# aleCombi/Hedgehog.jl

Hardware: AMD Instinct MI355X
Metric: MC path-steps/sec (Heston Euler-Maruyama, 1e6 paths x 252 steps per GPU) (higher is better)
Workload: dtype f64

## Files before the change

### hedgehog.jl_amd/csrc/hh_api.hip

```cpp
#include <cmath>
#include <cstdarg>
#include <cstdio>
#include <cstring>
#include <mutex>
#include <vector>

#include "hh_kernels.h"

#include "hh_ctx.h"

namespace {

const char* const kNoCtx = "hedgehog_mc: no context";

int ncomp_of(int dynamics) { return dynamics == HH_HESTON ? 2 : 1; }

constexpr uint64_t kMaxPaths = (1ull << 32) - 256;
constexpr uint32_t kMaxEulerSteps = 4u * 65535u;
constexpr uint32_t kMaxGridSteps = 65534u;

static bool bk_law_ok(const hh_model* m, double dt) {
  const double s2 = m->sigma * m->sigma;
  const double d = 4.0 * m->kappa * m->theta / s2;
  if (!(d >= 1e-8 && d <= 1e6)) return false;
  const double em1 = -std::expm1(-m->kappa * dt);
  const double lam_per_v = 4.0 * m->kappa * std::exp(-m->kappa * dt) / (s2 * em1);
  const double cscale = s2 * em1 / (4.0 * m->kappa);
  const double nuk = 4.0 * m->kappa * std::exp(-0.5 * m->kappa * dt) / s2 / em1;
  return std::isfinite(lam_per_v) && lam_per_v >= 0.0 && std::isfinite(cscale) && cscale > 0.0 &&
         std::isfinite(nuk) && nuk > 0.0 && std::isfinite(m->kappa * (1.0 + std::exp(-m->kappa * dt)) / em1);
}

int validate(hh_ctx* ctx, const hh_model* m, const hh_config* c) {
  if (!m || !c) return fail(ctx, HH_ERR_INVALID, "model/config is NULL");
  if (c->n_paths == 0) return fail(ctx, HH_ERR_INVALID, "n_paths must be >= 1");
  if (c->n_paths > kMaxPaths)
    return fail(ctx, HH_ERR_INVALID, "n_paths too large (max 2^32 - 256 per call; shard the ensemble)");
  if (c->strategy == HH_EULER_MARUYAMA && c->n_steps > kMaxEulerSteps)
    return fail(ctx, HH_ERR_INVALID, "n_steps too large (max %u)", kMaxEulerSteps);
  if (c->n_partials > HH_MAX_PARTIALS)
    return fail(ctx, HH_ERR_INVALID, "n_partials %u > HH_MAX_PARTIALS", c->n_partials);
  const bool logn = c->dynamics == HH_LOGNORMAL, hest = c->dynamics == HH_HESTON;
  if (!logn && !hest) return fail(ctx, HH_ERR_INVALID, "unknown dynamics %d", c->dynamics);
  const bool ok = (logn && (c->strategy == HH_EULER_MARUYAMA || c->strategy == HH_EXACT_LAW)) ||
                  (hest && (c->strategy == HH_EULER_MARUYAMA || c->strategy == HH_BROADIE_KAYA));
  if (!ok)
    return fail(ctx, HH_ERR_UNSUPPORTED, "no simulation method for dynamics %d with strategy %d",
                c->dynamics, c->strategy);
  if (!(m->S0 > 0.0) || !std::isfinite(m->S0)) return fail(ctx, HH_ERR_INVALID, "S0 must be > 0");
  if (!(m->T > 0.0) || !std::isfinite(m->T)) return fail(ctx, HH_ERR_INVALID, "T must be > 0");
  if (m->cp != 1.0 && m->cp != -1.0) return fail(ctx, HH_ERR_INVALID, "cp must be +1 or -1");
  if (hest && !(std::fabs(m->rho) <= 1.0)) return fail(ctx, HH_ERR_INVALID, "|rho| must be <= 1");
  if (!std::isfinite(m->sigma) || !std::isfinite(m->r_drift) || !std::isfinite(m->discount) ||
      !std::isfinite(m->strike) ||
      (hest && (!std::isfinite(m->V0) || !std::isfinite(m->kappa) || !std::isfinite(m->theta))))
    return fail(ctx, HH_ERR_INVALID, "model scalars must be finite");
  if (c->strategy == HH_EULER_MARUYAMA && c->n_steps == 0)
    return fail(ctx, HH_ERR_INVALID, "n_steps must be >= 1 for EulerMaruyama");
  if (c->strategy == HH_BROADIE_KAYA) {
    if (c->antithetic)
      return fail(ctx, HH_ERR_UNSUPPORTED, "HestonBroadieKaya has no antithetic form");
    if (c->n_partials)
      return fail(ctx, HH_ERR_UNSUPPORTED, "HestonBroadieKaya does not carry dual partials");
    if (m->sigma == 0.0 || m->kappa == 0.0 || !(m->V0 > 0.0))
      return fail(ctx, HH_ERR_INVALID, "HestonBroadieKaya needs sigma != 0, kappa != 0, V0 > 0");
    if ((c->bk_root_form != HH_BK_ROOT_SECANT && c->bk_root_form != HH_BK_ROOT_ORDER2) ||
        (c->bk_bracket_form != HH_BK_BRACKET_MIDPOINT && c->bk_bracket_form != HH_BK_BRACKET_ROOTS) ||
        (c->bk_caps != HH_BK_CAPS_AS_WRITTEN && c->bk_caps != HH_BK_CAPS_ROOTS_DEFAULT))
      return fail(ctx, HH_ERR_INVALID, "bk_root_form, bk_bracket_form, bk_caps: 0 or 1 each (hedgehog_mc.h)");
    if (!bk_law_ok(m, m->T))
      return fail(ctx, HH_ERR_INVALID, "HestonBroadieKaya needs 1e-8 <= d = 4 kappa theta / sigma^2 <= 1e6 "
                                       "(Bessel order d/2 - 1 strictly above -1, tables up to order 5e5) and "
                                       "finite transition constants (|kappa T| < 700)");
  }
  const bool euler = c->strategy == HH_EULER_MARUYAMA;
  if (c->noise_mode == HH_NOISE_REPLAY) {
    if (!c->replay) return fail(ctx, HH_ERR_INVALID, "REPLAY needs a replay buffer");
    if (((uintptr_t)c->replay & 15u) != 0)
      return fail(ctx, HH_ERR_INVALID, "replay buffer must be 16-byte aligned");
    if (c->replay_len) {
      uint64_t need = c->n_paths;
      if (c->strategy == HH_BROADIE_KAYA) need = 3 * c->n_paths;
// ... 320 lines not shown
    p.records = ctx->frecords;
    p.accum = accum_dev;
    fused_controls(ctx, p);
  }
  if (reduced) *reduced = fuse || bk;
  if (bk) {
    rc = ensure_bk_scratch(ctx, hh::bk_scratch_bytes(c->n_paths, ctx->bk_term_cache));
    if (rc) return rc;
    p.accum = accum_dev ? accum_dev : ctx->accum;
    p.bk_scratch = ctx->bk_scratch;
    p.bk_table_key = &ctx->bk_table_key;
    p.bk_term_cache = ctx->bk_term_cache;
    ctx->bk_last_n = c->n_paths;
    ctx->bk_last_cache = ctx->bk_term_cache;
  }

  if ((rc = stage_noise(ctx, c, p, false))) return rc;

  const size_t n_term = (size_t)c->n_paths * (c->antithetic ? 2 : 1);
  if (terminal && c->terminal_on_device) {
    p.terminal = terminal;
  } else if (terminal || need_terminal_dev) {
    rc = ensure(ctx, ctx->terminal, n_term);
    if (rc) return rc;
    p.terminal = ctx->terminal;
  }
  const int n_active = c->n_partials ? hh::count_active_partials(*m, *c) : 0;
  if (need_terminal_dev && n_active) {
    rc = ensure(ctx, ctx->terminal_d, n_term * (size_t)hh::pad_partials((uint32_t)n_active));
    if (rc) return rc;
    p.terminal_d = ctx->terminal_d;
  }
  if (terminal_dev_out) *terminal_dev_out = p.terminal;

  if (ctx->timing) HH_HIP(ctx, hipEventRecord(ctx->tev[ctx->t_count % hh_ctx::kTimingSlots][0], ctx->stream));
  if (c->strategy == HH_BROADIE_KAYA)
    HH_HIP(ctx, hh::launch_bk(*m, *c, p, ctx->stream));
  else
    HH_HIP(ctx, hh::launch_simulation(*m, *c, p, ctx->stream));
  return HH_OK;
}

static int end_timing(hh_ctx* ctx) {
  if (ctx->timing) {
    HH_HIP(ctx, hipEventRecord(ctx->tev[ctx->t_count % hh_ctx::kTimingSlots][1], ctx->stream));
    ++ctx->t_count;
  }
  return HH_OK;
}

static int copy_back_terminal(hh_ctx* ctx, const hh_config* c, double* terminal) {
  if (terminal && !c->terminal_on_device) {
    const size_t n_term = (size_t)c->n_paths * (c->antithetic ? 2 : 1);
    HH_HIP(ctx, hipMemcpyAsync(terminal, ctx->terminal, n_term * sizeof(double),
                               hipMemcpyDeviceToHost, ctx->stream));
    HH_HIP(ctx, hipStreamSynchronize(ctx->stream));
  }
  return HH_OK;
}

int hh_mc_accumulate(hh_ctx* ctx, const hh_model* m, const hh_config* c, double* accum_dev,
                     double* terminal) {
  if (!ctx) return HH_ERR_INVALID;
  std::lock_guard<std::recursive_mutex> lock__(ctx->mu);
  int rc = validate(ctx, m, c);
  if (rc) return rc;
  if (!accum_dev) return fail(ctx, HH_ERR_INVALID, "accum_dev is NULL");
  HH_HIP(ctx, hipSetDevice(ctx->device));
  bool reduced = false;
  rc = run_simulation(ctx, m, c, terminal, false, nullptr, accum_dev, &reduced);
  if (rc) return rc;
  if (!reduced)
    HH_HIP(ctx, hh::launch_reduce_records(ctx->records, hh::sim_records(*c), (double)c->n_paths, accum_dev, ctx->stream, 1, m, c));
  if ((rc = end_timing(ctx))) return rc;
  if ((rc = release_host_operands(ctx))) return rc;
  return copy_back_terminal(ctx, c, terminal);
}

static int next_pass(int remaining) {
  if (remaining <= hh::kMaxModelsPerPass) return remaining;
  return remaining == hh::kMaxModelsPerPass + 1 ? hh::kMaxModelsPerPass - 1 : hh::kMaxModelsPerPass;
}

int hh_mc_accumulate_multi(hh_ctx* ctx, const hh_model* models, uint32_t n_models, const hh_config* c,
                           double* accum_dev, double* const* terminals) {
  if (!ctx) return HH_ERR_INVALID;
  std::lock_guard<std::recursive_mutex> lock__(ctx->mu);
  if (!models || n_models == 0 || n_models > HH_MAX_MODELS)
    return fail(ctx, HH_ERR_INVALID, "hh_mc_accumulate_multi: 1 .. %d models", HH_MAX_MODELS);
  if (!accum_dev) return fail(ctx, HH_ERR_INVALID, "accum_dev is NULL");
  int rc;
  for (uint32_t k = 0; k < n_models; ++k)
    if ((rc = validate(ctx, &models[k], c))) return rc;
  if (c->n_partials)
    return fail(ctx, HH_ERR_UNSUPPORTED, "several models in one pass carry no dual partials (n_partials must be 0)");
  if (n_models == 1) return hh_mc_accumulate(ctx, models, c, accum_dev, terminals ? terminals[0] : nullptr);
  HH_HIP(ctx, hipSetDevice(ctx->device));
  if (c->strategy == HH_BROADIE_KAYA) {
    const uint32_t count = hh::bk_record_count(c->n_paths);
    if ((rc = ensure(ctx, ctx->records, 2 * (size_t)count * hh::kRecStride))) return rc;
    std::vector<int> leader(n_models, -1);
    for (uint32_t k = 0; k < n_models; ++k)
      for (uint32_t j = 0; j < k; ++j)
        if (leader[j] < 0 && hh::bk_same_chain(models[j], models[k])) {
          leader[k] = (int)j;
          break;
        }
    for (uint32_t k = 0; k < n_models; ++k) {
      if (leader[k] >= 0) continue;
      if ((rc = hh_mc_accumulate(ctx, &models[k], c, accum_dev + (size_t)k * HH_ACC_LEN, terminals ? terminals[k] : nullptr)))
        return rc;
      for (uint32_t f = k + 1; f < n_models; ++f) {
        if (leader[f] != (int)k) continue;
        double* terminal = terminals ? terminals[f] : nullptr;
        hh::DevicePtrs p{};
        p.records = ctx->records + (size_t)count * hh::kRecStride;
        p.bk_scratch = ctx->bk_scratch;
        p.bk_term_cache = ctx->bk_term_cache;
        if (terminal && c->terminal_on_device) {
          p.terminal = terminal;
        } else if (terminal) {
          if ((rc = ensure(ctx, ctx->terminal, (size_t)c->n_paths))) return rc;
          p.terminal = ctx->terminal;
        }
        if (ctx->timing) HH_HIP(ctx, hipEventRecord(ctx->tev[ctx->t_count % hh_ctx::kTimingSlots][0], ctx->stream));
        HH_HIP(ctx, hh::launch_bk_refinish(models[f], *c, p, ctx->records, ctx->stream));
        HH_HIP(ctx, hh::launch_reduce_records(p.records, count, (double)c->n_paths, accum_dev + (size_t)f * HH_ACC_LEN,
                                              ctx->stream, 1, &models[f], c, false,
                                              hh::bk_live_records(ctx->bk_scratch, c->n_paths)));
        if ((rc = end_timing(ctx))) return rc;
        if ((rc = copy_back_terminal(ctx, c, terminal))) return rc;
      }
    }
    return HH_OK;
  }
  const uint32_t n_tiles = hh::tiles_for(c->n_paths);
  const size_t rec_elems = (size_t)n_tiles * hh::kRecStride;
  const bool fuse = fuse_for(ctx, c);
  if (fuse) rc = ensure_poisoned(ctx, (size_t)n_models * rec_elems);
  else rc = ensure(ctx, ctx->records, (size_t)n_models * rec_elems);
  if (rc) return rc;
  hh::DevicePtrs base{};
  if (fuse) fused_controls(ctx, base);
  if ((rc = stage_noise(ctx, c, base, true))) return rc;
  const size_t n_term = (size_t)c->n_paths * (c->antithetic ? 2 : 1);
  bool any_host_terminal = false;
  if (terminals && !c->terminal_on_device) {
    for (uint32_t k = 0; k < n_models; ++k) any_host_terminal = any_host_terminal || terminals[k] != nullptr;
    if (any_host_terminal && (rc = ensure(ctx, ctx->terminal, (size_t)n_models * n_term))) return rc;
  }
  std::vector<hh::DevicePtrs> p(n_models, base);
  for (uint32_t k = 0; k < n_models; ++k) {
    p[k].records = (fuse ? ctx->frecords : ctx->records) + (size_t)k * rec_elems;
    p[k].accum = fuse ? accum_dev + (size_t)k * HH_ACC_LEN : nullptr;
    double* t = terminals ? terminals[k] : nullptr;
    p[k].terminal = !t ? nullptr : c->terminal_on_device ? t : ctx->terminal + (size_t)k * n_term;
  }
  if (ctx->timing) HH_HIP(ctx, hipEventRecord(ctx->tev[ctx->t_count % hh_ctx::kTimingSlots][0], ctx->stream));
  for (uint32_t k0 = 0; k0 < n_models;) {
    const int take = next_pass((int)(n_models - k0));
    HH_HIP(ctx, hh::launch_simulation_multi(models + k0, take, *c, p.data() + k0, ctx->stream));
    if (!fuse)
      for (int k = 0; k < take; ++k)
        HH_HIP(ctx, hh::launch_reduce_records(p[k0 + k].records, hh::sim_records(*c), (double)c->n_paths,
                                              accum_dev + (size_t)(k0 + k) * HH_ACC_LEN, ctx->stream, 1, &models[k0 + k], c));
    k0 += (uint32_t)take;
  }
  if ((rc = end_timing(ctx))) return rc;
  if ((rc = release_host_operands(ctx))) return rc;
  if (any_host_terminal) {
    for (uint32_t k = 0; k < n_models; ++k)
      if (terminals[k])
        HH_HIP(ctx, hipMemcpyAsync(terminals[k], p[k].terminal, n_term * sizeof(double), hipMemcpyDeviceToHost, ctx->stream));
    HH_HIP(ctx, hipStreamSynchronize(ctx->stream));
  }
  return HH_OK;
}

int hh_mc_solve_multi(hh_ctx* ctx, const hh_model* models, uint32_t n_models, const hh_config* c, hh_result* out,
                      double* const* terminals) {
  if (!ctx) return HH_ERR_INVALID;
  std::lock_guard<std::recursive_mutex> lock__(ctx->mu);
  if (!out || !models || n_models == 0 || n_models > HH_MAX_MODELS)
    return fail(ctx, HH_ERR_INVALID, "hh_mc_solve_multi: 1 .. %d models and their results", HH_MAX_MODELS);
  const WallClock clock;
  HH_HIP(ctx, hipSetDevice(ctx->device));
  const size_t n_acc = (size_t)n_models * HH_ACC_LEN;
  int rc = ensure(ctx, ctx->basket_accum, n_acc);
  if (rc) return rc;
  HH_HIP(ctx, hipEventRecord(ctx->ev0, ctx->stream));
  if ((rc = hh_mc_accumulate_multi(ctx, models, n_models, c, ctx->basket_accum, terminals))) return rc;
  HH_HIP(ctx, hipEventRecord(ctx->ev1, ctx->stream));
  double host[HH_MAX_MODELS * HH_ACC_LEN];
  HH_HIP(ctx, hipMemcpyAsync(host, ctx->basket_accum, n_acc * sizeof(double), hipMemcpyDeviceToHost, ctx->stream));
  HH_HIP(ctx, hipStreamSynchronize(ctx->stream));
  double kernel_ms, total_ms;
  if ((rc = solve_times(ctx, clock, &kernel_ms, &total_ms))) return rc;
  rc = finalize_results(models, 1, c, host, n_models, kernel_ms, total_ms, out);
  return rc ? finalize_failed(ctx, rc) : HH_OK;
}

int hh_mc_accumulate_basket(hh_ctx* ctx, const hh_model* m, const hh_config* c,
                            const double* strikes, const double* cps, uint32_t n_payoffs,
                            double* accum_dev, double* terminal) {
  if (!ctx) return HH_ERR_INVALID;
  std::lock_guard<std::recursive_mutex> lock__(ctx->mu);
  int rc = validate(ctx, m, c);
  if (rc) return rc;
  if (!accum_dev || !strikes || !cps || n_payoffs == 0 || n_payoffs > 65535)
    return fail(ctx, HH_ERR_INVALID, "hh_mc_accumulate_basket: bad arguments");
  for (uint32_t k = 0; k < n_payoffs; ++k)
    if (cps[k] != 1.0 && cps[k] != -1.0) return fail(ctx, HH_ERR_INVALID, "cp must be +1 or -1");
  if (m->dstrike)
    return fail(ctx, HH_ERR_UNSUPPORTED, "strike partials are not carried through a basket");
  HH_HIP(ctx, hipSetDevice(ctx->device));
  double* term_dev = nullptr;
  rc = run_simulation(ctx, m, c, terminal, true, &term_dev);
  if (rc) return rc;

  hh::BasketArgs b{};
  b.n_paths = c->n_paths;
  b.n_chunks = hh::basket_chunks(c->n_paths);
  b.antithetic = c->antithetic;
  std::vector<double> payoffs(strikes, strikes + n_payoffs);
  payoffs.insert(payoffs.end(), cps, cps + n_payoffs);
  const double* payoffs_dev = nullptr;
  rc = stage_host(ctx, ctx->payoffs, payoffs.size(), payoffs.data(), payoffs.size(), &payoffs_dev);
  if (rc) return rc;
  rc = ensure(ctx, ctx->basket_records, (size_t)n_payoffs * b.n_chunks * hh::kRecStride);
  if (rc) return rc;
  b.terminal = term_dev;
  const int n_active = c->n_partials ? hh::count_active_partials(*m, *c) : 0;
  b.terminal_d = n_active ? ctx->terminal_d : nullptr;
  b.strikes = payoffs_dev;
  b.cps = payoffs_dev + n_payoffs;
  b.records = ctx->basket_records;
  HH_HIP(ctx, hh::launch_basket_payoffs(b, n_payoffs, (uint32_t)n_active, ctx->stream));
  HH_HIP(ctx, hh::launch_reduce_records(ctx->basket_records, b.n_chunks, (double)c->n_paths,
                                        accum_dev, ctx->stream, n_payoffs, m, c, true));
  if (c->strategy == HH_BROADIE_KAYA)
    HH_HIP(ctx, hh::launch_copy_bk_counters(ctx->accum, accum_dev, n_payoffs, ctx->stream));
  if ((rc = end_timing(ctx))) return rc;
  if ((rc = release_host_operands(ctx))) return rc;
  return copy_back_terminal(ctx, c, terminal);
}

int hh_mc_solve_basket(hh_ctx* ctx, const hh_model* m, const hh_config* c, const double* strikes,
                       const double* cps, uint32_t n_payoffs, hh_result* out, double* terminal) {
  if (!ctx) return HH_ERR_INVALID;
// ... 1033 lines not shown
```

### hedgehog.jl_amd/csrc/hh_kernels.h

```cpp
#pragma once
#include <hip/hip_runtime.h>
#include <stdint.h>

#include "../../include/hedgehog_mc.h"
#include "hh_layout.h"

namespace hh {

constexpr int kRecStride = HH_ACC_LEN;
constexpr unsigned long long kPoison = 0x7FF8C0DE7FF8C0DEull;
constexpr unsigned long long kFinishSpinTicksDefault = 500000000ull;
constexpr int kRecItmS = 11;

template <int P>
struct DualT {
  double v;
  double d[P > 0 ? P : 1];
};

constexpr int kMaxBasis = 4;
enum { kBasisV0 = 0, kBasisKappa = 1, kBasisTheta = 2, kBasisSigma = 3 };
struct PartialMap {
  int sim;
  int n;
// ... 5 lines not shown
};
template <int P>
struct SimArgs {
  DualT<P> x0;
  DualT<P> v0;
  DualT<P> kappa, theta, sigma;
  DualT<P> r;
  DualT<P> gdrift;
  DualT<P> strike;
  DualT<P> law_mu, law_sd;
  double dt, sqrt_dt, rho, rho_c, cp;
  uint64_t n_paths;
  uint64_t path_offset;
  uint32_t n_steps;
  uint32_t n_tiles;
  uint32_t tail_from;
  const uint64_t* seeds;
  const double* replay;
  double* terminal;
  double* terminal_d;
  double* records;
  double* accum;
  double acc_n_paths;
  unsigned int* finish_state;
  unsigned long long finish_spin_ticks;
  uint32_t reducer_tile;
  PartialMap map;
};

struct DevicePtrs {
  const uint64_t* seeds;
  const double* replay;
  double* terminal;
  double* terminal_d;
  double* records;
  double* accum;
  unsigned int* finish_state;
  long long finish_spin_ticks = -1;
  int finish_tile_first = 0;
  void* bk_scratch;
  struct BkTableKey* bk_table_key;
  int bk_term_cache;
  void* bk_sort;
  bool replay_path_major;
};
inline bool replay_direct_path_major(uint32_t n_steps, int ncomp) { return ((uint64_t)n_steps * ncomp) % 2 == 0; }
struct BkTableKey {
  const void* where;
  double nu;
  double kappa, sigma2, T;
};

constexpr int kBasketChunk = 4096;
struct BasketArgs {
  const double* terminal;
  const double* terminal_d;
  const double* strikes;
  const double* cps;
  uint64_t n_paths;
  uint32_t n_chunks;
  int antithetic;
  double* records;
};
inline uint32_t basket_chunks(uint64_t n_paths) {
  return (uint32_t)((n_paths + kBasketChunk - 1) / kBasketChunk);
}

constexpr int kExactPairs = 8, kExactPairsHuge = 64;
constexpr int kExactPairsSmall = 4;
int exact_pairs_per_lane(uint64_t n_paths);
inline uint32_t exact_records(uint64_t n_paths) {
  const uint64_t per = 512ull * (uint64_t)exact_pairs_per_lane(n_paths);
  return (uint32_t)((n_paths + per - 1) / per);
}
inline uint32_t sim_records(const hh_config& c) {
  return c.strategy == HH_EXACT_LAW ? exact_records(c.n_paths) : tiles_for(c.n_paths);
}
inline int pad_partials(uint32_t p) { return p <= 4 ? (int)p : 4; }

int launch_simulation(const hh_model& m, const hh_config& c, const DevicePtrs& p, hipStream_t s);
int launch_simulation_multi(const hh_model* models, int n_models, const hh_config& c, const DevicePtrs* p,
                            hipStream_t s);
constexpr int kMaxModelsPerPass = 4;
SimArgs<0> make_args0(const hh_model& m, const hh_config& c, const DevicePtrs& p);
struct BkTransition {
  const double* in_spot;
  const double* in_var;
  double* out_spot;
  double* out_var;
  uint32_t step;
};
bool bk_same_chain(const hh_model& a, const hh_model& b);
int launch_bk_refinish(const hh_model& m, const hh_config& c, const DevicePtrs& p, const double* rec0, hipStream_t s);
int launch_bk(const hh_model& m, const hh_config& c, const DevicePtrs& p, hipStream_t s,
              const BkTransition* tr = nullptr, bool upload_tables = true);
int launch_bk_grid(const hh_model& m, const hh_config& c, const DevicePtrs& p, hipStream_t s,
                   double* spot_rows, double* var_rows, uint32_t k0, uint32_t n_dates, bool upload_tables);
uint32_t bk_grid_dates_per_chain(uint64_t n_paths, uint32_t n_steps);
size_t bk_grid_sort_bytes(uint64_t n_chain);
size_t bk_scratch_bytes(uint64_t n_paths, int term_cache = 0);
void bk_diag_ptrs(const void* scratch, uint64_t n_paths, int term_cache, const uint32_t** decisions,
                  const uint32_t** series_len);
uint32_t bk_record_count(uint64_t n_paths);
const uint32_t* bk_live_records(const void* scratch, uint64_t n_paths);
int launch_copy_bk_counters(const double* src, double* accum, uint32_t n_groups, hipStream_t s);
int launch_fill_rows(double* spot0, double* var0, uint64_t n, double S0, double V0, hipStream_t s);
int launch_reduce_records(const double* records, uint32_t n_records, double n_paths, double* accum,
                          hipStream_t s, uint32_t n_groups = 1, const hh_model* m = nullptr,
                          const hh_config* c = nullptr, bool basket = false,
                          const uint32_t* n_records_dev = nullptr);
int count_active_partials(const hh_model& m, const hh_config& c);
int launch_basket_payoffs(const BasketArgs& b, uint32_t n_payoffs, uint32_t n_active_partials,
                          hipStream_t s);
constexpr uint32_t kCarrMadanMaxSubpanels = 1024;
uint32_t carr_madan_subpanels(double alpha, double bound);
int launch_carr_madan(const hh_model& m, int dynamics, int compat_sqrt_alpha, double alpha,
                      double bound, double* out_dev, hipStream_t s);
int launch_carr_madan_grad(const hh_model& m, int dynamics, int compat_sqrt_alpha, double alpha,
                           double bound, const double* per_payoff_dev, uint32_t n_payoffs,
                           double* out_dev, hipStream_t s);
int launch_carr_madan_basket(const hh_model& m, int dynamics, int compat_sqrt_alpha, double alpha,
                             double bound, const double* per_payoff_dev, uint32_t n_payoffs,
                             double* out_dev, hipStream_t s);
struct CrrTree {
  double F, K, cp, u, p, q, disc;
  int32_t style;
  uint32_t row;
};
int launch_crr(const CrrTree* trees_dev, const double* spot_factors_dev, int steps, uint32_t n_trees,
               double* out_dev, hipStream_t s);
struct FdOption {
  double S0, K, cp, r, T;
  double h, x0;
  double lo, di, up;
  int32_t style;
  int32_t pad_;
};
int launch_fd(const FdOption* opts_dev, int space_steps, int time_steps, int rannacher_steps, uint32_t n_options,
              double* out_dev, hipStream_t s);
uint32_t lsm_chunks(uint64_t ntot);
size_t lsm_scratch_doubles(uint64_t ntot, uint32_t n_steps, int degree);
enum { kLsmPhaseStats = 0, kLsmPhasePow = 1, kLsmPhaseInit = 2, kLsmPhaseStep = 3, kLsmPhaseFinal = 4 };
int launch_lsm_phase(int phase, uint32_t t, const double* grid, uint64_t ntot, uint32_t n_steps,
                     double strike, double cp, double step_discount, int degree, int32_t* tau,
                     double* val, double* scratch, double* records, const double* vec_in,
                     double* vec_out, hipStream_t s);
int launch_gbm_grid(const uint64_t* seeds_dev, uint64_t n_paths, uint32_t n_steps, double S0,
                    double r, double sigma, double T, int anti, double* grid, hipStream_t s);
int launch_euler_grid(const hh_model& m, const hh_config& c, const uint64_t* seeds_dev, bool log_state,
                      double* grid, double* var_grid, hipStream_t s);
int launch_path_stats(const hh_model& m, const hh_config& c, const uint64_t* seeds_dev, uint32_t monitor_every,
                      bool include_start, bool bridge, double* stats, hipStream_t s);
struct PathPayoffArgs {
  const double* stats;
  const hh_path_payoff* payoffs;
  double* values;
  double* records;
  double n_mon;
  uint64_t n_paths;
  uint32_t n_chunks;
  int antithetic;
  int extremes;
};
int launch_path_payoffs(const PathPayoffArgs& b, uint32_t n_payoffs, hipStream_t s);
double merton_compensator(const hh_jump& jump);
constexpr int kMertonPerLane = 8;
// ... 22 lines not shown
```

### hedgehog.jl_amd/csrc/hh_multi.hip

```cpp
#include <type_traits>

#include "hh_sim.h"

namespace hh {

template <int K>
struct MultiArgs {
  SimArgs<0> m[K];
};

constexpr int kMultiChunk = 4;
constexpr int kMultiMaxWaves = 3;

template <class M, bool REPLAY, bool ANTI, int K, bool SHARED>
__global__ __launch_bounds__(kTile)
__attribute__((amdgpu_waves_per_eu(1, REPLAY ? kMultiMaxWaves : 8))) void euler_multi_kernel(const MultiArgs<K> a) {
  constexpr int NC = M::NCOMP;
  using State = typename M::State;
  const SimArgs<0>& a0 = a.m[0];
  const uint32_t tile = blockIdx.x, tid = threadIdx.x;
  const uint64_t path = (uint64_t)tile * kTile + tid;
  const uint32_t n_steps = a0.n_steps;

  State st[K];
  State sa[ANTI ? K : 1];
#pragma unroll
  for (int k = 0; k < K; ++k) {
    M::init(st[k], a.m[k]);
    if constexpr (ANTI) M::init(sa[k], a.m[k]);
  }
  auto step_all = [&](double d1, double d2) {
#pragma unroll
    for (int k = 0; k < K; ++k) {
      M::step(st[k], a.m[k], d1, d2);
      if constexpr (ANTI) M::step(sa[k], a.m[k], -d1, -d2);
    }
  };

  if constexpr (REPLAY) {
    const double* __restrict__ base = a0.replay + (size_t)tile * n_steps * NC * kTile + tid;
    constexpr int CH = kMultiChunk;
    double X[CH][NC], Y[CH][NC];
    auto ld = [&](double(&buf)[CH][NC], uint32_t s0) {
#pragma unroll
      for (int u = 0; u < CH; ++u) {
        if (s0 + u < n_steps) {
#pragma unroll
          for (int c = 0; c < NC; ++c) buf[u][c] = stream_load(base + ((size_t)(s0 + u) * NC + c) * kTile);
        }
      }
    };
    auto go = [&](const double(&buf)[CH][NC], uint32_t s0) {
#pragma unroll
      for (int u = 0; u < CH; ++u)
        if (s0 + u < n_steps) step_all(buf[u][0], NC > 1 ? buf[u][NC - 1] : 0.0);
    };
    auto ldf = [&](double(&buf)[CH][NC], uint32_t s0) {
#pragma unroll
      for (int u = 0; u < CH; ++u)
#pragma unroll
        for (int c = 0; c < NC; ++c) buf[u][c] = stream_load(base + ((size_t)(s0 + u) * NC + c) * kTile);
    };
    auto gof = [&](const double(&buf)[CH][NC]) {
#pragma unroll
      for (int u = 0; u < CH; ++u) step_all(buf[u][0], NC > 1 ? buf[u][NC - 1] : 0.0);
    };
    uint32_t s = 0;
    if (n_steps >= 2u * CH) {
      ldf(X, 0);
      while (s + 3u * CH <= n_steps) {
        ldf(Y, s + CH);
        gof(X);
        ldf(X, s + 2u * CH);
        gof(Y);
        s += 2u * CH;
      }
      ld(Y, s + CH);
      gof(X);
      s += CH;
      ld(X, s + CH);
      go(Y, s);
      go(X, s + CH);
    } else {
      ld(X, 0);
      while (s < n_steps) {
        ld(Y, s + CH);
        go(X, s);
        s += CH;
        if (s >= n_steps) break;
        ld(X, s + CH);
        go(Y, s);
        s += CH;
      }
    }
  } else {
    const uint64_t key = path < a0.n_paths ? a0.seeds[path] : 0ull;
    if constexpr (NC == 2) {
      for (uint32_t s = 0; s < n_steps; ++s) {
        double z1, z2;
        normal_pair(key, s, 0u, 0u, kDomEuler, z1, z2);
        if constexpr (SHARED) {
          step_all(a0.sqrt_dt * z1, a0.sqrt_dt * fma(a0.rho, z1, a0.rho_c * z2));
        } else {
#pragma unroll
          for (int k = 0; k < K; ++k) {
            const double d1 = a.m[k].sqrt_dt * z1;
            const double d2 = a.m[k].sqrt_dt * fma(a.m[k].rho, z1, a.m[k].rho_c * z2);
            M::step(st[k], a.m[k], d1, d2);
            if constexpr (ANTI) M::step(sa[k], a.m[k], -d1, -d2);
          }
        }
      }
    } else {
      auto one = [&](double z) {
#pragma unroll
        for (int k = 0; k < K; ++k) {
          const double d = a.m[k].sqrt_dt * z;
          M::step(st[k], a.m[k], d, 0.0);
          if constexpr (ANTI) M::step(sa[k], a.m[k], -d, 0.0);
        }
      };
      for (uint32_t s = 0; s < n_steps; s += 2) {
        double z1, z2;
        normal_pair(key, s >> 1, 0u, 0u, kDomEuler, z1, z2);
        one(z1);
        if (s + 1 < n_steps) one(z2);
      }
    }
  }

#pragma unroll
  for (int k = 0; k < K; ++k) {
    double acc[4] = {0.0, 0.0, 0.0, 0.0};
    finish_path<0, ANTI>(st[k], sa[ANTI ? k : 0], a.m[k], path, acc);
    if (k) __syncthreads();
    block_reduce_publish<4, kTile / 64, 2>(acc, a.m[k].records + (size_t)tile * kRecStride, a.m[k].accum != nullptr, false);
  }
  if (a0.accum && reduces_records(tile, a0)) {
#pragma unroll
    for (int k = 0; k < K; ++k) {
      if (k) __syncthreads();
      finish_records<kTile, 0>(a.m[k]);
    }
  }
}

template <bool REPLAY, bool ANTI, int K, int PAIRS>
__global__ __launch_bounds__(kTile) void exact_multi_kernel(const MultiArgs<K> a) {
  const SimArgs<0>& a0 = a.m[0];
  const uint32_t chunk = blockIdx.x, tid = threadIdx.x;
  struct S {
    DualT<0> x;
  };
  double acc[K][4];
#pragma unroll
  for (int k = 0; k < K; ++k)
#pragma unroll
    for (int i = 0; i < 4; ++i) acc[k][i] = 0.0;
#pragma unroll 2
  for (int jp = 0; jp < PAIRS; ++jp) {
    const uint64_t path0 = ((uint64_t)chunk * PAIRS + jp) * (2 * kTile) + (uint64_t)tid * 2;
    double z[2];
    exact_pair_normals<REPLAY>(a0, path0, z);
#pragma unroll
    for (int k = 0; k < K; ++k) {
#pragma unroll
      for (int j = 0; j < 2; ++j) {
        S st, sa;
        st.x.v = fma(a.m[k].law_sd.v, z[j], a.m[k].law_mu.v);
        if constexpr (ANTI) sa.x.v = 2 * a.m[k].law_mu.v - st.x.v;
        finish_path<0, ANTI>(st, sa, a.m[k], path0 + j, acc[k]);
      }
    }
  }
#pragma unroll
  for (int k = 0; k < K; ++k) {
    if (k) __syncthreads();
    block_reduce_publish<4, kTile / 64, 2>(acc[k], a.m[k].records + (size_t)chunk * kRecStride, a.m[k].accum != nullptr, false);
  }
  if (a0.accum && reduces_records(chunk, a0)) {
#pragma unroll
    for (int k = 0; k < K; ++k) {
      if (k) __syncthreads();
      finish_records<kTile, 0>(a.m[k]);
    }
  }
}


template <class M, bool REPLAY, bool ANTI, int K>
static int launch_multi_k(const MultiArgs<K>& a, bool shared, hipStream_t s) {
  const dim3 g(a.m[0].n_tiles), b(kTile);
  if constexpr (!REPLAY && M::NCOMP == 2) {
    if (shared) {
      hipLaunchKernelGGL((euler_multi_kernel<M, REPLAY, ANTI, K, true>), g, b, 0, s, a);
      return (int)hipGetLastError();
    }
  }
  hipLaunchKernelGGL((euler_multi_kernel<M, REPLAY, ANTI, K, false>), g, b, 0, s, a);
  return (int)hipGetLastError();
}

template <class M, int K>
static int launch_multi_m(const MultiArgs<K>& a, bool replay, bool anti, bool shared, hipStream_t s) {
  if (replay) return anti ? launch_multi_k<M, true, true, K>(a, shared, s) : launch_multi_k<M, true, false, K>(a, shared, s);
  return anti ? launch_multi_k<M, false, true, K>(a, shared, s) : launch_multi_k<M, false, false, K>(a, shared, s);
}

template <int K>
static int launch_multi(const hh_model* models, const hh_config& c, const DevicePtrs* p, hipStream_t s) {
  MultiArgs<K> a;
  bool shared = true;
  for (int k = 0; k < K; ++k) {
    a.m[k] = make_args0(models[k], c, p[k]);
    shared = shared && a.m[k].rho == a.m[0].rho && a.m[k].dt == a.m[0].dt;
  }
  const bool anti = c.antithetic != 0, replay = c.noise_mode == HH_NOISE_REPLAY;
  if (c.strategy == HH_EXACT_LAW) {
    const dim3 g(a.m[0].n_tiles), b(kTile);
    auto pick = [&](auto replay_c, auto anti_c) {
      constexpr bool R = decltype(replay_c)::value, A = decltype(anti_c)::value;
      const int pairs = exact_pairs_per_lane(c.n_paths);
      return pairs == kExactPairsHuge ? exact_multi_kernel<R, A, K, kExactPairsHuge>
             : pairs == kExactPairs   ? exact_multi_kernel<R, A, K, kExactPairs>
                                      : exact_multi_kernel<R, A, K, kExactPairsSmall>;
    };
    using T = std::true_type;
    using F = std::false_type;
    auto kernel = replay ? (anti ? pick(T{}, T{}) : pick(T{}, F{})) : (anti ? pick(F{}, T{}) : pick(F{}, F{}));
    hipLaunchKernelGGL(kernel, g, b, 0, s, a);
    return (int)hipGetLastError();
  }
  if (c.dynamics == HH_LOGNORMAL) return launch_multi_m<GbmModel<0>, K>(a, replay, anti, shared, s);
  if (c.em_split) return launch_multi_m<HestonModel<0, true>, K>(a, replay, anti, shared, s);
  return launch_multi_m<HestonModel<0, false>, K>(a, replay, anti, shared, s);
}

int launch_simulation_multi(const hh_model* models, int n_models, const hh_config& c, const DevicePtrs* p,
                            hipStream_t s) {
  switch (n_models) {
    case 2: return launch_multi<2>(models, c, p, s);
    case 3: return launch_multi<3>(models, c, p, s);
    case 4: return launch_multi<4>(models, c, p, s);
    default: return (int)hipErrorInvalidValue;
  }
}

}
```

### hedgehog.jl_amd/csrc/hh_sim.h

```cpp
#pragma once
#include <type_traits>

#include "hh_kernels.h"
#include "hh_reduce.h"
#include "hh_rng.h"

namespace hh {


__device__ __forceinline__ double sqrt_clipped(double w) {
  const double y = __builtin_fmin(__builtin_amdgcn_rsq(w), 0x1p1000);
  double g = w * y, h = 0.5 * y;
  const double r = fma(-h, g, 0.5);
  g = fma(g, r, g);
  h = fma(h, r, h);
  g = fma(fma(-g, g, w), h, g);
  return fma(fma(-g, g, w), h, g);
}

template <int P, bool SPLIT>
struct HestonModel {
  static constexpr int NCOMP = 2;
  struct State {
    DualT<P> x, v;
  };
  __device__ static __forceinline__ void init(State& s, const SimArgs<P>& a) {
    s.x = a.x0;
    s.v = a.v0;
  }
  __device__ static __forceinline__ void step(State& s, const SimArgs<P>& a, double dW1,
                                              double dW2) {
    double g;
    step(s, a, dW1, dW2, g);
  }
  __device__ static __forceinline__ void step(State& s, const SimArgs<P>& a, double dW1, double dW2, double& g) {
    const bool pos = s.v.v > 0.0;
    double vp;
    asm("v_max_f64 %0, %1, 0" : "=v"(vp) : "v"(s.v.v));
    const double th_m_v = a.theta.v - vp;
    const double Kx = fma(a.dt, fma(-0.5, vp, a.r.v), s.x.v);
    const double Kv = fma(a.dt, a.kappa.v * th_m_v, s.v.v);
    const bool wpos = SPLIT ? (Kv > 0.0) : pos;
    const double w = SPLIT ? (wpos ? Kv : 0.0) : vp;
    const double sq = sqrt_clipped(w);
    if constexpr (P > 0) {
      double inv2s = 0.0;
      if (wpos) {
        const double r0 = __builtin_amdgcn_rcp(sq);
        inv2s = 0.5 * fma(r0, fma(-sq, r0, 1.0), r0);
      }
      const double A = a.dt * th_m_v, B = sq * dW2;
      const double m = pos ? 1.0 - a.dt * a.kappa.v : 1.0;
      const double h = pos ? 0.5 * a.dt : 0.0;
      const double e1 = inv2s * dW1;
      const double se2 = (a.sigma.v * inv2s) * dW2;
#pragma unroll
      for (int k = 0; k < P; ++k) {
        const double dv = s.v.d[k];
        const double f = fma(a.kappa.d[k], A, (a.dt * a.kappa.v) * a.theta.d[k]);
        const double Kvd = fma(m, dv, f);
        const double x0 = s.x.d[k] + a.dt * a.r.d[k];
        if constexpr (SPLIT) {
          s.x.d[k] = fma(e1, Kvd, fma(-h, dv, x0));
          s.v.d[k] = fma(se2, Kvd, fma(a.sigma.d[k], B, Kvd));
        } else {
          s.x.d[k] = fma(e1 - h, dv, x0);
          s.v.d[k] = fma(se2, dv, fma(a.sigma.d[k], B, Kvd));
        }
      }
    }
    s.x.v = fma(sq, dW1, Kx);
    s.v.v = fma(a.sigma.v * sq, dW2, Kv);
    g = sq;
  }
};

template <int P>
struct GbmModel {
  static constexpr int NCOMP = 1;
  struct State {
    DualT<P> x;
  };
  __device__ static __forceinline__ void init(State& s, const SimArgs<P>& a) { s.x = a.x0; }
  __device__ static __forceinline__ void step(State& s, const SimArgs<P>& a, double dW, double) {
    if constexpr (P > 0) {
#pragma unroll
      for (int k = 0; k < P; ++k)
        s.x.d[k] = fma(a.sigma.d[k], dW, fma(a.dt, a.gdrift.d[k], s.x.d[k]));
    }
    s.x.v = fma(a.sigma.v, dW, fma(a.dt, a.gdrift.v, s.x.v));
  }
  __device__ static __forceinline__ void step(State& s, const SimArgs<P>& a, double dW, double, double& g) {
    step(s, a, dW, 0.0);
    g = a.sigma.v;
  }
};


template <int P>
__device__ __forceinline__ void euler_pair_increments(uint64_t key, uint32_t s, const SimArgs<P>& a, double& d1,
                                                      double& d2) {
  double z1, z2;
  normal_pair(key, s, 0u, 0u, kDomEuler, z1, z2);
  d1 = a.sqrt_dt * z1;
  d2 = a.sqrt_dt * fma(a.rho, z1, a.rho_c * z2);
}
__device__ __forceinline__ void euler_scalar_normals(uint64_t key, uint32_t h, double& z1, double& z2) {
  normal_pair(key, h, 0u, 0u, kDomEuler, z1, z2);
}

__device__ __forceinline__ void euler_bridge_draws(uint64_t key, uint32_t k, double& L1, double& L2) {
  const Philox4 b = philox4x32_10(k, 0u, 0u, kDomBridge, (uint32_t)key, (uint32_t)(key >> 32));
  L1 = neg2_log_unit(u01_fast(b.c0, b.c1));
  L2 = neg2_log_unit(u01_fast(b.c2, b.c3));
}


template <int P>
__device__ __forceinline__ void payoff_of(const DualT<P>& x, const SimArgs<P>& a, double& S,
                                          double& p, double (&pd)[P > 0 ? P : 1], double& wS,
                                          double& wN) {
  S = exp(x.v);
  const double m = a.cp * (S - a.strike.v);
  const bool itm = m > 0.0;
  p = itm ? m : 0.0;
  wS = itm ? a.cp * S : 0.0;
  wN = itm ? a.cp : 0.0;
  if constexpr (P > 0) {
#pragma unroll
    for (int k = 0; k < P; ++k) pd[k] = wS * x.d[k];
  }
}

template <int N, int NWAVES, int TAIL = 0>
__device__ __forceinline__ void block_reduce_store(double (&acc)[N], double* __restrict__ rec) {
#pragma unroll
  for (int i = 0; i < N; ++i) {
#pragma unroll
    for (int off = 32; off > 0; off >>= 1) acc[i] += __shfl_down(acc[i], off, 64);
  }
  __shared__ double sm[NWAVES][N];
  const int lane = threadIdx.x & 63, wave = threadIdx.x >> 6;
  if (lane == 0) {
#pragma unroll
    for (int i = 0; i < N; ++i) sm[wave][i] = acc[i];
  }
  __syncthreads();
  if (threadIdx.x == 0) {
#pragma unroll
    for (int i = 0; i < kRecStride; ++i) rec[i] = 0.0;
#pragma unroll
    for (int i = 0; i < N; ++i) {
      double t = sm[0][i];
#pragma unroll
      for (int w = 1; w < NWAVES; ++w) t += sm[w][i];
      rec[i < N - TAIL ? i : kRecItmS + (i - (N - TAIL))] = t;
// ... 294 lines not shown
```

Before: 436.9 billion.

## Share one variance path across multi-model Heston passes with identical variance parameters

Adds a shared-variance kernel variant: when all models in a pass share v0, kappa, theta, sigma and dt (plus rho and noise when not replaying), the variance process is stepped once and only the log-spot update runs per model. Host-side pass planning groups models with identical variance processes into the same pass and sends single leftovers to the single-model kernel. This removes redundant sqrt and variance arithmetic per model per step, at the cost of more kernel instantiations, a tighter waves-per-EU bound for the replay variant, and a different pass partition.

```diff
diff --git a/hedgehog.jl_amd/csrc/hh_api.hip b/hedgehog.jl_amd/csrc/hh_api.hip
--- a/hedgehog.jl_amd/csrc/hh_api.hip
+++ b/hedgehog.jl_amd/csrc/hh_api.hip
@@ -1,3 +1,4 @@
+#include <algorithm>
 #include <cmath>
 #include <cstdarg>
 #include <cstdio>
@@ -484,6 +485,42 @@
   return remaining == hh::kMaxModelsPerPass + 1 ? hh::kMaxModelsPerPass - 1 : hh::kMaxModelsPerPass;
 }
 
+static std::vector<std::vector<uint32_t>> plan_passes(const hh_model* models, uint32_t n_models, const hh_config* c) {
+  using Pass = std::vector<uint32_t>;
+  auto cut = [](const Pass& of, std::vector<Pass>& into) {
+    for (size_t k0 = 0; k0 < of.size();) {
+      const size_t take = (size_t)next_pass((int)(of.size() - k0));
+      into.emplace_back(of.begin() + (long)k0, of.begin() + (long)(k0 + take));
+      k0 += take;
+    }
+  };
+  std::vector<Pass> groups;
+  for (uint32_t k = 0; k < n_models; ++k) {
+    size_t g = 0;
+    while (g < groups.size() && !hh::euler_same_variance(models[groups[g][0]], models[k], *c)) ++g;
+    if (g == groups.size()) groups.emplace_back();
+    groups[g].push_back(k);
+  }
+  std::vector<Pass> shared;
+  Pass pool;
+  for (const Pass& g : groups) {
+    if (g.size() >= 2) cut(g, shared);
+    else pool.push_back(g[0]);
+  }
+  const size_t at_most = (n_models + hh::kMaxModelsPerPass - 1) / hh::kMaxModelsPerPass;
+  for (;;) {
+    std::vector<Pass> passes = shared;
+    std::sort(pool.begin(), pool.end());
+    cut(pool, passes);
+    if (passes.size() <= at_most || shared.empty()) return passes;
+    size_t least = 0;
+    for (size_t i = 1; i < shared.size(); ++i)
+      if (shared[i].size() <= shared[least].size()) least = i;
+    pool.insert(pool.end(), shared[least].begin(), shared[least].end());
+    shared.erase(shared.begin() + (long)least);
+  }
+}
+
 int hh_mc_accumulate_multi(hh_ctx* ctx, const hh_model* models, uint32_t n_models, const hh_config* c,
                            double* accum_dev, double* const* terminals) {
   if (!ctx) return HH_ERR_INVALID;
@@ -559,14 +596,21 @@
     p[k].terminal = !t ? nullptr : c->terminal_on_device ? t : ctx->terminal + (size_t)k * n_term;
   }
   if (ctx->timing) HH_HIP(ctx, hipEventRecord(ctx->tev[ctx->t_count % hh_ctx::kTimingSlots][0], ctx->stream));
-  for (uint32_t k0 = 0; k0 < n_models;) {
-    const int take = next_pass((int)(n_models - k0));
-    HH_HIP(ctx, hh::launch_simulation_multi(models + k0, take, *c, p.data() + k0, ctx->stream));
+  for (const std::vector<uint32_t>& pass : plan_passes(models, n_models, c)) {
+    hh_model pass_models[hh::kMaxModelsPerPass];
+    hh::DevicePtrs pass_ptrs[hh::kMaxModelsPerPass];
+    for (size_t k = 0; k < pass.size(); ++k) {
+      pass_models[k] = models[pass[k]];
+      pass_ptrs[k] = p[pass[k]];
+    }
+    if (pass.size() == 1)
+      HH_HIP(ctx, hh::launch_simulation(pass_models[0], *c, pass_ptrs[0], ctx->stream));
+    else
+      HH_HIP(ctx, hh::launch_simulation_multi(pass_models, (int)pass.size(), *c, pass_ptrs, ctx->stream));
     if (!fuse)
-      for (int k = 0; k < take; ++k)
-        HH_HIP(ctx, hh::launch_reduce_records(p[k0 + k].records, hh::sim_records(*c), (double)c->n_paths,
-                                              accum_dev + (size_t)(k0 + k) * HH_ACC_LEN, ctx->stream, 1, &models[k0 + k], c));
-    k0 += (uint32_t)take;
+      for (uint32_t k : pass)
+        HH_HIP(ctx, hh::launch_reduce_records(p[k].records, hh::sim_records(*c), (double)c->n_paths,
+                                              accum_dev + (size_t)k * HH_ACC_LEN, ctx->stream, 1, &models[k], c));
   }
   if ((rc = end_timing(ctx))) return rc;
   if ((rc = release_host_operands(ctx))) return rc;
diff --git a/hedgehog.jl_amd/csrc/hh_kernels.h b/hedgehog.jl_amd/csrc/hh_kernels.h
--- a/hedgehog.jl_amd/csrc/hh_kernels.h
+++ b/hedgehog.jl_amd/csrc/hh_kernels.h
@@ -111,6 +111,7 @@
 int launch_simulation_multi(const hh_model* models, int n_models, const hh_config& c, const DevicePtrs* p,
                             hipStream_t s);
 constexpr int kMaxModelsPerPass = 4;
+bool euler_same_variance(const hh_model& a, const hh_model& b, const hh_config& c);
 SimArgs<0> make_args0(const hh_model& m, const hh_config& c, const DevicePtrs& p);
 struct BkTransition {
   const double* in_spot;
diff --git a/hedgehog.jl_amd/csrc/hh_multi.hip b/hedgehog.jl_amd/csrc/hh_multi.hip
--- a/hedgehog.jl_amd/csrc/hh_multi.hip
+++ b/hedgehog.jl_amd/csrc/hh_multi.hip
@@ -1,3 +1,4 @@
+#include <cstring>
 #include <type_traits>
 
 #include "hh_sim.h"
@@ -11,10 +12,13 @@
 
 constexpr int kMultiChunk = 4;
 constexpr int kMultiMaxWaves = 3;
-
-template <class M, bool REPLAY, bool ANTI, int K, bool SHARED>
+constexpr int kMultiSharedMaxWaves = 2;
+
+template <class M, bool REPLAY, bool ANTI, int K, bool SHARED, bool SHV>
 __global__ __launch_bounds__(kTile)
-__attribute__((amdgpu_waves_per_eu(1, REPLAY ? kMultiMaxWaves : 8))) void euler_multi_kernel(const MultiArgs<K> a) {
+__attribute__((amdgpu_waves_per_eu(1, REPLAY ? (SHV && !ANTI ? kMultiSharedMaxWaves : kMultiMaxWaves) : 8))) void euler_multi_kernel(
+    const MultiArgs<K> a) {
+  static_assert(!SHV || (M::NCOMP == 2 && (REPLAY || SHARED)), "one variance process: Heston, on increments formed once");
   constexpr int NC = M::NCOMP;
   using State = typename M::State;
   const SimArgs<0>& a0 = a.m[0];
@@ -30,10 +34,21 @@
     if constexpr (ANTI) M::init(sa[k], a.m[k]);
   }
   auto step_all = [&](double d1, double d2) {
-#pragma unroll
-    for (int k = 0; k < K; ++k) {
-      M::step(st[k], a.m[k], d1, d2);
-      if constexpr (ANTI) M::step(sa[k], a.m[k], -d1, -d2);
+    if constexpr (SHV) {
+      const auto f = M::step_v(st[0], a0, d2);
+#pragma unroll
+      for (int k = 0; k < K; ++k) M::step_x(st[k], a.m[k], f, d1);
+      if constexpr (ANTI) {
+        const auto fa = M::step_v(sa[0], a0, -d2);
+#pragma unroll
+        for (int k = 0; k < K; ++k) M::step_x(sa[k], a.m[k], fa, -d1);
+      }
+    } else {
+#pragma unroll
+      for (int k = 0; k < K; ++k) {
+        M::step(st[k], a.m[k], d1, d2);
+        if constexpr (ANTI) M::step(sa[k], a.m[k], -d1, -d2);
+      }
     }
   };
 
@@ -188,34 +203,60 @@
 }
 
 
+template <class M>
+constexpr bool kHasVariance = false;
+template <bool SPLIT>
+constexpr bool kHasVariance<HestonModel<0, SPLIT>> = true;
+
 template <class M, bool REPLAY, bool ANTI, int K>
-static int launch_multi_k(const MultiArgs<K>& a, bool shared, hipStream_t s) {
+static int launch_multi_k(const MultiArgs<K>& a, bool shared, bool shv, hipStream_t s) {
   const dim3 g(a.m[0].n_tiles), b(kTile);
+  if constexpr (kHasVariance<M>) {
+    if (shv) {
+      hipLaunchKernelGGL((euler_multi_kernel<M, REPLAY, ANTI, K, !REPLAY, true>), g, b, 0, s, a);
+      return (int)hipGetLastError();
+    }
+  }
   if constexpr (!REPLAY && M::NCOMP == 2) {
     if (shared) {
-      hipLaunchKernelGGL((euler_multi_kernel<M, REPLAY, ANTI, K, true>), g, b, 0, s, a);
+      hipLaunchKernelGGL((euler_multi_kernel<M, REPLAY, ANTI, K, true, false>), g, b, 0, s, a);
       return (int)hipGetLastError();
     }
   }
-  hipLaunchKernelGGL((euler_multi_kernel<M, REPLAY, ANTI, K, false>), g, b, 0, s, a);
+  hipLaunchKernelGGL((euler_multi_kernel<M, REPLAY, ANTI, K, false, false>), g, b, 0, s, a);
   return (int)hipGetLastError();
 }
 
 template <class M, int K>
-static int launch_multi_m(const MultiArgs<K>& a, bool replay, bool anti, bool shared, hipStream_t s) {
-  if (replay) return anti ? launch_multi_k<M, true, true, K>(a, shared, s) : launch_multi_k<M, true, false, K>(a, shared, s);
-  return anti ? launch_multi_k<M, false, true, K>(a, shared, s) : launch_multi_k<M, false, false, K>(a, shared, s);
+static int launch_multi_m(const MultiArgs<K>& a, bool replay, bool anti, bool shared, bool shv, hipStream_t s) {
+  if (replay) return anti ? launch_multi_k<M, true, true, K>(a, shared, shv, s) : launch_multi_k<M, true, false, K>(a, shared, shv, s);
+  return anti ? launch_multi_k<M, false, true, K>(a, shared, shv, s) : launch_multi_k<M, false, false, K>(a, shared, shv, s);
+}
+
+static bool same_bits(double x, double y) { return std::memcmp(&x, &y, sizeof x) == 0; }
+static bool same_variance_process(const SimArgs<0>& x, const SimArgs<0>& y, bool replay) {
+  const bool same = same_bits(x.v0.v, y.v0.v) && same_bits(x.kappa.v, y.kappa.v) && same_bits(x.theta.v, y.theta.v) &&
+                    same_bits(x.sigma.v, y.sigma.v) && same_bits(x.dt, y.dt);
+  if (replay) return same;
+  return same && same_bits(x.rho, y.rho) && same_bits(x.rho_c, y.rho_c) && same_bits(x.sqrt_dt, y.sqrt_dt);
+}
+
+bool euler_same_variance(const hh_model& x, const hh_model& y, const hh_config& c) {
+  if (c.strategy != HH_EULER_MARUYAMA || c.dynamics == HH_LOGNORMAL) return false;
+  const DevicePtrs none{};
+  return same_variance_process(make_args0(x, c, none), make_args0(y, c, none), c.noise_mode == HH_NOISE_REPLAY);
 }
 
 template <int K>
 static int launch_multi(const hh_model* models, const hh_config& c, const DevicePtrs* p, hipStream_t s) {
   MultiArgs<K> a;
-  bool shared = true;
+  const bool anti = c.antithetic != 0, replay = c.noise_mode == HH_NOISE_REPLAY;
+  bool shared = true, shv = true;
   for (int k = 0; k < K; ++k) {
     a.m[k] = make_args0(models[k], c, p[k]);
     shared = shared && a.m[k].rho == a.m[0].rho && a.m[k].dt == a.m[0].dt;
-  }
-  const bool anti = c.antithetic != 0, replay = c.noise_mode == HH_NOISE_REPLAY;
+    shv = shv && same_variance_process(a.m[0], a.m[k], replay);
+  }
   if (c.strategy == HH_EXACT_LAW) {
     const dim3 g(a.m[0].n_tiles), b(kTile);
     auto pick = [&](auto replay_c, auto anti_c) {
@@ -231,9 +272,9 @@
     hipLaunchKernelGGL(kernel, g, b, 0, s, a);
     return (int)hipGetLastError();
   }
-  if (c.dynamics == HH_LOGNORMAL) return launch_multi_m<GbmModel<0>, K>(a, replay, anti, shared, s);
-  if (c.em_split) return launch_multi_m<HestonModel<0, true>, K>(a, replay, anti, shared, s);
-  return launch_multi_m<HestonModel<0, false>, K>(a, replay, anti, shared, s);
+  if (c.dynamics == HH_LOGNORMAL) return launch_multi_m<GbmModel<0>, K>(a, replay, anti, shared, false, s);
+  if (c.em_split) return launch_multi_m<HestonModel<0, true>, K>(a, replay, anti, shared, shv, s);
+  return launch_multi_m<HestonModel<0, false>, K>(a, replay, anti, shared, shv, s);
 }
 
 int launch_simulation_multi(const hh_model* models, int n_models, const hh_config& c, const DevicePtrs* p,
diff --git a/hedgehog.jl_amd/csrc/hh_sim.h b/hedgehog.jl_amd/csrc/hh_sim.h
--- a/hedgehog.jl_amd/csrc/hh_sim.h
+++ b/hedgehog.jl_amd/csrc/hh_sim.h
@@ -72,6 +72,27 @@
     s.x.v = fma(sq, dW1, Kx);
     s.v.v = fma(a.sigma.v * sq, dW2, Kv);
     g = sq;
+  }
+  struct Diffusion {
+    double vp, sq;
+  };
+  __device__ static __forceinline__ Diffusion step_v(State& s, const SimArgs<P>& a, double dW2) {
+    static_assert(P == 0, "the split step carries no partials");
+    const bool pos = s.v.v > 0.0;
+    double vp;
+    asm("v_max_f64 %0, %1, 0" : "=v"(vp) : "v"(s.v.v));
+    const double th_m_v = a.theta.v - vp;
+    const double Kv = fma(a.dt, a.kappa.v * th_m_v, s.v.v);
+    const bool wpos = SPLIT ? (Kv > 0.0) : pos;
+    const double w = SPLIT ? (wpos ? Kv : 0.0) : vp;
+    const double sq = sqrt_clipped(w);
+    s.v.v = fma(a.sigma.v * sq, dW2, Kv);
+    return {vp, sq};
+  }
+  __device__ static __forceinline__ void step_x(State& s, const SimArgs<P>& a, const Diffusion& d, double dW1) {
+    static_assert(P == 0, "the split step carries no partials");
+    const double Kx = fma(a.dt, fma(-0.5, d.vp, a.r.v), s.x.v);
+    s.x.v = fma(d.sq, dW1, Kx);
   }
 };
 
```

Result: slower. 427.8 billion (-2.1%).
